# elavoie/non-iid-topology-simulator

Hardware: AMD Instinct MI355X
Metric: param-GB/s mixed (device-resident), 1000-node d-cliques, P=1M fp32 (higher is better)
Workload: dtype f32; 1 GPU; d-cliques N=1000 (10 cliques x 100, fully-connected interclique, MH weights; topology generated by the reference, seed 1337); n_nodes=1000, p=1048576, kernel=clique, mode=fast, parallelism=single GPU, halo_rows_rank0=0, hipgraph=False, slab_memory=VMM 2 MiB chunks (niidmix_hbm_alloc), slab_layout=column-blocked [1024, 1000, 1024], clique-contiguous rows

## Files before the change

include/niidmix.h:

```cpp
#ifndef NIIDMIX_H
#define NIIDMIX_H

#include <stdint.h>
#include <sys/types.h>

#ifdef __cplusplus
extern "C" {
#endif

#define NIIDMIX_ABI_VERSION 6

enum niidmix_status {
    NIIDMIX_OK = 0,
    NIIDMIX_EINVAL = 1,
    NIIDMIX_EALIAS = 2,
    NIIDMIX_EHIP = 3,
    NIIDMIX_EUNSUPPORTED = 4
};

enum niidmix_mode {
    NIIDMIX_MODE_EXACT = 0,
    NIIDMIX_MODE_FAST = 1
};

#define NIIDMIX_FLAG_AVERAGE_ONLY 2

#define NIIDMIX_FLAG_LOW_DEGREE 4

#define NIIDMIX_FLAG_MEAN 8

int niidmix_abi_version(void);

const char *niidmix_last_error(void);

int niidmix_mix_csr_f32(const float *x, int64_t ld_x, float *y, int64_t ld_y, int64_t n_rows,
                        int64_t p, const int64_t *row_ptr, const int32_t *col, const float *val,
                        int mode, void *stream);

int niidmix_mix_ell_f32(const float *x, int64_t ld_x, float *y, int64_t ld_y, int64_t n_rows,
                        int64_t p, int k, const int32_t *ell_col, const float *ell_val,
                        const int32_t *ell_len, int mode, void *stream);

int niidmix_mix_band_f32(const float *x, int64_t ld_x, float *y, int64_t ld_y, int64_t n_rows,
                         int64_t p, int k, int band, const int32_t *ell_col, const float *ell_val,
// ... 174 lines not shown
```

non-iid-topology-simulator_amd/csrc/niidmix.hip:

```cpp
#include <hip/hip_runtime.h>
#include <rccl/rccl.h>

#include <dlfcn.h>
#include <stdarg.h>
#include <stdlib.h>
#include <stdint.h>
#include <stdio.h>
#include <string.h>
#include <sys/types.h>

#include <mutex>
#include <unordered_map>
#include <type_traits>
#include <vector>

#include "../../include/niidmix.h"

typedef float floatx16 __attribute__((ext_vector_type(16)));

namespace {

thread_local char g_last_error[512] = "";

int set_error(int code, const char *fmt, ...) {
// ... 2377 lines not shown
#define NIIDMIX_SEG_REMOTE NIIDMIX_SEG_REMOTE_M("0xfff")
#define NIIDMIX_SEG_REMOTE8 NIIDMIX_SEG_REMOTE_M("7")
#define NIIDMIX_SEG_REMOTE_M(MASK)                                                                   \
    "s_bitcmp1_b32 s41, 29\n\t"                                                                     \
    "s_cbranch_scc0 .Lw_lds_%=\n\t"                                                                 \
    "s_and_b32 s46, s41, " MASK "\n\t"                                                              \
    "s_lshl_b32 s46, s46, 1\n\t"                                                                    \
    "s_set_gpr_idx_on s46, gpr_idx(SRC0)\n\t"                                                       \
    "v_mov_b32 %[q0], v64\n\t"                                                                      \
    "v_mov_b32 %[q1], v65\n\t"                                                                      \
    "s_set_gpr_idx_off\n\t"                                                                         \
    "s_branch .Lw_mskgo_%=\n"                                                                       \
    ".Lw_lds_%=:\n\t"
#define NIIDMIX_REM_IN , [rem] "{v[64:95]}"(rem)
#define NIIDMIX_REM_IN8 , [rem] "{v[64:79]}"(rem)
#define NIIDMIX_SEG_WALK(UPD, MSK) NIIDMIX_SEG_WALK_X(UPD, MSK, "", )
#define NIIDMIX_SEG_LOOP(S, UPD)                                                                     \
    ".Lseg_loop" S "_%=:\n\t"                                                                       \
    NIIDMIX_SEG_POS("%[x0]", "%[x2]", "o2", S "0", UPD)                                              \
    NIIDMIX_SEG_POS("%[x1]", "%[x3]", "o3", S "1", UPD)                                              \
    NIIDMIX_SEG_POS("%[x2]", "%[x0]", "o4", S "2", UPD)                                              \
    NIIDMIX_SEG_POS("%[x3]", "%[x1]", "o5", S "3", UPD)                                              \
    "v_add_u32 %[va], %[o4], %[va]\n\t"                                                             \
    "s_branch .Lseg_loop" S "_%=\n\t"                                                               \
    NIIDMIX_SEG_SKIPBLK("%[x0]", S "0", UPD)                                                         \
    NIIDMIX_SEG_SKIPBLK("%[x1]", S "1", UPD)                                                         \
    NIIDMIX_SEG_SKIPBLK("%[x2]", S "2", UPD)                                                         \
    NIIDMIX_SEG_SKIPBLK("%[x3]", S "3", UPD)
#define NIIDMIX_SEG_WALK_X(UPD, MSK, RMSK, RIN)                                                      \
    asm volatile("s_mov_b32 s36, %[sb0]\n"                                                           \
                 ".Lc_next_%=:\n\t"                                                                  \
                 "s_cmp_ge_u32 s36, %[sb1]\n\t"                                                      \
                 "s_cbranch_scc1 .Lw_end_%=\n\t"                                                     \
                 "s_sub_u32 s37, %[sb1], s36\n\t"                                                    \
                 "s_min_u32 s37, s37, 64\n\t"                                                        \
                 "s_sub_u32 s35, s37, 1\n\t"                                                         \
                 "v_min_u32 %[vo], %[ln], s35\n\t"                                                   \
                 "v_add_u32 %[vo], s36, %[vo]\n\t"                                                   \
                 "v_lshlrev_b32 %[vo], 4, %[vo]\n\t"                                                 \
                 "global_load_dword %[dx], %[vo], %[sp]\n\t"                                         \
                 "global_load_dword %[dy], %[vo], %[sp] offset:4\n\t"                                \
                 "global_load_dword %[dz], %[vo], %[sp] offset:8\n\t"                                \
                 "s_waitcnt vmcnt(0)\n\t"                                                            \
                 "s_mov_b32 s40, 0\n"                                                                \
                 ".Lw_next_%=:\n\t"                                                                  \
                 "s_cmp_ge_u32 s40, s37\n\t"                                                         \
                 "s_cbranch_scc1 .Lc_done_%=\n\t"                                                    \
                 "v_readlane_b32 s41, %[dx], s40\n\t"                                                \
                 "v_readlane_b32 s42, %[dy], s40\n\t"                                                \
                 "v_readlane_b32 s43, %[dz], s40\n\t"                                                \
                 "s_add_u32 s40, s40, 1\n\t"                                                         \
                 "s_and_b32 s39, s41, 0xfff\n\t"                                                     \
                 "s_mul_i32 s39, s39, %[o1]\n\t"                                                     \
                 "s_add_u32 s39, s39, %[base]\n\t"                                                   \
                 "v_add_u32 %[va], s39, %[l8]\n\t"                                                   \
                 "s_bitcmp1_b32 s41, 30\n\t"                                                         \
                 "s_cbranch_scc1 .Lw_masked_%=\n\t"                                                  \
// ... 31 lines not shown
                 NIIDMIX_SEG_LOOP("n14", UPD##14)                                                    \
                 NIIDMIX_SEG_LOOP("n15", UPD##15)                                                    \
                 NIIDMIX_SEG_LOOP("h", UPD##8)                                                       \
                 NIIDMIX_SEG_LOOP("q", UPD##4)                                                       \
                 "\n.Lw_masked_%=:\n\t"                                                              \
                 RMSK                                                                                \
                 "ds_read_b32 %[q0], %[va]\n\t"                                                      \
                 "ds_read_b32 %[q1], %[va] offset:4\n\t"                                             \
                 "s_waitcnt lgkmcnt(0)\n"                                                             \
                 ".Lw_mskgo_%=:\n\t"                                                                 \
                 MSK                                                                                 \
                 "\n.Lc_done_%=:\n\t"                                                                \
                 "s_add_u32 s36, s36, 64\n\t"                                                        \
                 "s_branch .Lc_next_%=\n"                                                            \
                 ".Lw_end_%=:\n\t"                                                                   \
                 "s_waitcnt lgkmcnt(0)"                                                              \
                 : "+{v[32:63]}"(acc), [x0] "=&v"(x0), [x1] "=&v"(x1), [x2] "=&v"(x2),             \
                   [x3] "=&v"(x3), [pr] "=&v"(pr), [sv] "=&v"(sv),                                   \
                   [q0] "=&v"(q0), [q1] "=&v"(q1), [va] "=&v"(va), [dx] "=&v"(dx), [dy] "=&v"(dy),  \
                   [dz] "=&v"(dz), [vo] "=&v"(vo)                                                   \
                 : [sp] "s"(segp), [sb0] "s"(sb0), [sb1] "s"(sb1), [ln] "v"(lane), [base] "s"(base), \
                   [w0] "s"(w0), [w1] "s"(w1), [l8] "v"(lane8), [nr] "s"(nr), [o1] "i"(RB),            \
                   [o2] "i"(2 * RB), [o3] "i"(3 * RB), [o4] "i"(4 * RB), [o5] "i"(5 * RB) RIN         \
                 : "s35", "s36", "s37", "s38", "s39", "s40", "s41", "s42", "s43", "s44", "s45", "s46", \
                   "s47", "m0", "scc", "memory")
template <bool EXACT, int RB>
__device__ __forceinline__ void tlds16_walk(Acc16 &acc, const int32_t *segp, int sb0, int sb1, int base,
                                            int w0, int w1, int lane8, int lane, int nr) {
    static_assert(5 * RB < 65536, "ds_read immediate offset");
    uint64_t x0, x1, x2, x3, pr;
    uint64_t sv;
    uint32_t q0, q1, va, dx, dy, dz, vo;
    if constexpr (EXACT) NIIDMIX_SEG_WALK(NIIDMIX_SEG_UPD_EXACT, NIIDMIX_MSK_EXACT);
    else NIIDMIX_SEG_WALK(NIIDMIX_UPD_FAST, NIIDMIX_MSK_FAST);
    (void)pr;
}
typedef float Rem32 __attribute__((ext_vector_type(32)));
typedef float Rem16 __attribute__((ext_vector_type(16)));
template <int NREM> struct RemRegs { typedef Rem32 V; };
template <> struct RemRegs<8> { typedef Rem16 V; };
template <bool EXACT, int RB, int NREM>
__device__ __forceinline__ void tlds16_walk_rem(Acc16 &acc, const int32_t *segp, int sb0, int sb1,
                                                int base, int w0, int w1, int lane8, int lane,
                                                int nr, const typename RemRegs<NREM>::V &rem) {
    static_assert(5 * RB < 65536, "ds_read immediate offset");
    static_assert(NREM == 8 || NREM == 16, "8 or 16 register rows");
    uint64_t x0, x1, x2, x3, pr;
    uint64_t sv;
    uint32_t q0, q1, va, dx, dy, dz, vo;
    if constexpr (EXACT && NREM == 16)
        NIIDMIX_SEG_WALK_X(NIIDMIX_SEG_UPD_EXACT, NIIDMIX_MSK_EXACT, NIIDMIX_SEG_REMOTE, NIIDMIX_REM_IN);
    else if constexpr (NREM == 16)
        NIIDMIX_SEG_WALK_X(NIIDMIX_UPD_FAST, NIIDMIX_MSK_FAST, NIIDMIX_SEG_REMOTE, NIIDMIX_REM_IN);
    else if constexpr (EXACT)
        NIIDMIX_SEG_WALK_X(NIIDMIX_SEG_UPD_EXACT, NIIDMIX_MSK_EXACT, NIIDMIX_SEG_REMOTE8, NIIDMIX_REM_IN8);
    else
        NIIDMIX_SEG_WALK_X(NIIDMIX_UPD_FAST, NIIDMIX_MSK_FAST, NIIDMIX_SEG_REMOTE8, NIIDMIX_REM_IN8);
    (void)pr;
}

template <bool EXACT>
__device__ __forceinline__ void tlds16_init(Acc16 &acc, int d_slot, int d_ws, int rb, int base, int lane8) {
    uint64_t x0, x1, t, pr;
    uint32_t va;
    if constexpr (EXACT)
        asm volatile("s_mov_b64 s[46:47], 0\n\t"
                 "v_readlane_b32 s40, %[ds], 0\n\t""v_readlane_b32 s42, %[dw], 0\n\t""s_mul_i32 s40, s40, %[rb]\n\t""s_add_u32 s40, s40, %[base]\n\t""v_add_u32 %[va], s40, %[l8]\n\t""ds_read_b64 %[x0], %[va]\n\t"
                 "v_readlane_b32 s40, %[ds], 1\n\t""v_readlane_b32 s44, %[dw], 1\n\t""s_mul_i32 s40, s40, %[rb]\n\t""s_add_u32 s40, s40, %[base]\n\t""v_add_u32 %[va], s40, %[l8]\n\t""ds_read_b64 %[x1], %[va]\n\t"
                 "s_waitcnt lgkmcnt(1)\n\t""v_pk_mul_f32 %[t], %[x0], s[46:47]\n\t""v_pk_mul_f32 %[pr], %[x0], s[42:43] op_sel_hi:[1,0]\n\t""v_pk_add_f32 v[32:33], %[t], %[pr]\n\t"
                 "v_readlane_b32 s40, %[ds], 2\n\t""v_readlane_b32 s42, %[dw], 2\n\t""s_mul_i32 s40, s40, %[rb]\n\t""s_add_u32 s40, s40, %[base]\n\t""v_add_u32 %[va], s40, %[l8]\n\t""ds_read_b64 %[x0], %[va]\n\t"
                 "s_waitcnt lgkmcnt(1)\n\t""v_pk_mul_f32 %[t], %[x1], s[46:47]\n\t""v_pk_mul_f32 %[pr], %[x1], s[44:45] op_sel_hi:[1,0]\n\t""v_pk_add_f32 v[34:35], %[t], %[pr]\n\t"
                 "v_readlane_b32 s40, %[ds], 3\n\t""v_readlane_b32 s44, %[dw], 3\n\t""s_mul_i32 s40, s40, %[rb]\n\t""s_add_u32 s40, s40, %[base]\n\t""v_add_u32 %[va], s40, %[l8]\n\t""ds_read_b64 %[x1], %[va]\n\t"
// ... 101 lines not shown
#endif
#ifndef NIIDMIX_MF_SPLIT
#define NIIDMIX_MF_SPLIT 0
#endif
#ifndef NIIDMIX_TLDS_GLDS
#define NIIDMIX_TLDS_GLDS 1
#endif
inline size_t tlds_slack(bool seg, int cw) {
    const size_t spare = seg ? 2 * (size_t)cw * sizeof(float) : 0;
    return NIIDMIX_TLDS_GLDS && spare < 1024 ? 1024 - spare : 0;
}
constexpr int tile_lds_max_waves(int rt) { return rt == 8 ? 16 : rt == 16 ? 12 : 4; }

template <bool B> struct BoolC { static constexpr bool value = B; };

template <bool EXACT, int RT, int SV, int RS, bool SEG, int NREM = 0, bool MF = false, bool REM2 = false>
__global__ __launch_bounds__(64 * tile_lds_max_waves(RT)) void k_mix_tile_lds(
    const float *__restrict__ x, int64_t ld_x, float *__restrict__ y, int64_t ld_y, int64_t p,
    int64_t n_grp, const int32_t *__restrict__ grp_tile_ptr, const int32_t *__restrict__ grp_src_ptr,
    const int32_t *__restrict__ grp_src_rows, const int64_t *__restrict__ sub_ptr,
    const int32_t *__restrict__ sub_rows, const int32_t *__restrict__ sub_slot,
    const float *__restrict__ sub_wself, const int32_t *__restrict__ pos_slot,
    const uint32_t *__restrict__ pos_mask, const float *__restrict__ pos_w, int tl_flags,
    const int32_t *__restrict__ seg_ptr, const int32_t *__restrict__ seg,
    const float *__restrict__ seg_w, const int32_t *__restrict__ mf_ptr,
    const int32_t *__restrict__ mf, int mf_waves, const int32_t *__restrict__ rem_rows) {
    constexpr int rs = RS;
    const bool avg_only = (tl_flags & 1) != 0;
    const bool small_loops = (tl_flags & 2) == 0;
    constexpr int64_t CW = 2 * RS;
    constexpr uint32_t FULL = (uint32_t)((1ull << RT) - 1ull);
// ... 295 lines not shown
#pragma unroll
            for (int r = 0; r < RT; ++r) {
                const f2 xs = stage[__builtin_amdgcn_readlane(d_slot, r) * rs + sl];
                const float ws = __int_as_float(__builtin_amdgcn_readlane(__float_as_int(d_ws), r));
                acc.set(r, axpy2<EXACT>(ws, xs, xs * 0.f));
            }
        }
        if constexpr (SEG && RT == 16 && NIIDMIX_TLDS_ASM && (NIIDMIX_TLDS_SPLIT == 0 || NIIDMIX_TLDS_SPLIT == 2)) {
            {
                const int sb0 = seg_ptr[sub], sb1 = seg_ptr[sub + 1];
                const int w0 = __float_as_int(seg_w[2 * sub]), w1 = __float_as_int(seg_w[2 * sub + 1]);
                const uint64_t used = __ballot(lane < RT && d_row >= 0);
                const int hi = used ? 64 - __builtin_clzll(used) : 1;
                const int nr = __builtin_amdgcn_readfirstlane(
                    !small_loops ? 16 : hi <= 4 ? 4 : hi <= 8 ? 8 : hi);
                if constexpr (REM && REM2) {
                    int sm = sb1;
                    for (int b = sb0; b < sb1; b += kWave) {
                        const int i = b + lane;
                        const int dx = i < sb1 ? seg[4 * i] : 0;
                        const uint64_t hit = __ballot((dx & (3 << 29)) == (3 << 29) && (dx & 0xfff) >= 8);
                        if (hit) { sm = b + __builtin_ctzll(hit); break; }
                    }
                    tlds16_walk_rem<EXACT, rs * (int)sizeof(f2), 8>(acc.v[0], seg, sb0, sm, (int)lds_base,
                                                                     w0, w1, lane8, lane, nr, rem);
                    if (sm < sb1) {
                        const int sl_ = lane < rs ? lane : rs - 1;
                        const int64_t cr = c0 + 2 * sl_ < p ? c0 + 2 * sl_ : c0;
#pragma unroll
                        for (int r = 0; r < 8; ++r) {
                            const int row = rem_rows[sub * 16 + 8 + r];
// ... 1821 lines not shown
    const int64_t n_chunks = (p + cw - 1) / cw;
    const int64_t n_sub_groups = (plan->n_sub + 3) / 4;
    const int64_t n_items = n_sub_groups * ((n_chunks + 7) / 8) * 8;
    auto kfn = pick<true, false>(mode == NIIDMIX_MODE_EXACT, [&](auto E) { return pick<8, 16, 32>(plan->rt, [&](auto R) {
        return pick<4, 2>(ne, [&](auto N) { return pick<4, 2, 1>(vw, [&](auto V) {
            return k_mix_tile<E(), V(), V() == 4 ? 4 : N(), R()>; }); }); }); });
    hipLaunchKernelGGL(kfn, dim3((unsigned)grid_for(n_items)), dim3(256), 0, s, x, ld_x, y, ld_y, p,
                       plan->n_sub, plan->sub_ptr, plan->sub_rows, plan->sub_wself, plan->pos_src,
                       plan->pos_mask, plan->pos_w, n_sub_groups, n_items, avg_only);
    return check_launch("k_mix_tile");
}

int niidmix_mix_tile_lds_f32(const float *x, int64_t ld_x, float *y, int64_t ld_y, int64_t n_rows,
                             int64_t p, const niidmix_tile_lds_plan *plan, int mode, void *stream) {
    if (!plan) return set_error(NIIDMIX_EINVAL, "null plan");
    int avg_only = strip_flags(&mode, NIIDMIX_FLAG_AVERAGE_ONLY) ? 1 : 0;
    if (int rc = check_mode(mode)) return rc;
    if (env_int("NIIDMIX_TLDS_SMALL", 1) == 0) avg_only |= 2;
    if (p < 0 || plan->n_grp < 0) return set_error(NIIDMIX_EINVAL, "negative size");
    if (plan->rt != 8 && plan->rt != 16 && plan->rt != 32)
        return set_error(NIIDMIX_EUNSUPPORTED, "tile of %d rows (8, 16 or 32 supported)", plan->rt);
    if (plan->n_grp == 0 || p == 0) return NIIDMIX_OK;
    if (!x || !y || !plan->grp_tile_ptr || !plan->grp_src_ptr || !plan->grp_src_rows ||
        !plan->sub_ptr || !plan->sub_rows || !plan->sub_slot || !plan->sub_wself ||
        !plan->pos_slot || !plan->pos_mask || !plan->pos_w)
        return set_error(NIIDMIX_EINVAL, "null pointer");
    if (int rc = check_ld(ld_x, ld_y, p)) return rc;
    if (ld_x >= (1LL << 30)) return set_error(NIIDMIX_EUNSUPPORTED, "ld_x >= 2^30");
    if (n_rows < 1) return set_error(NIIDMIX_EINVAL, "n_rows < 1");
    if (int rc = check_overlap(x, ld_x, y, ld_y, n_rows, p)) return rc;
    if (plan->max_src < 1 || plan->max_src > 256)
        return set_error(NIIDMIX_EUNSUPPORTED, "group with %d source rows (1..256 supported)", plan->max_src);
    const int max_waves = tile_lds_max_waves(plan->rt);
    if (plan->max_tiles < 1 || plan->max_tiles > max_waves)
        return set_error(NIIDMIX_EUNSUPPORTED, "group with %d tiles of %d rows (1..%d supported)",
                         plan->max_tiles, plan->rt, max_waves);
    if (vec_width({p, ld_x, ld_y}, {x, y}) == 1)
        return set_error(NIIDMIX_EUNSUPPORTED, "LDS tile kernel needs even p, ld and 8-B aligned slabs");
    const int sv = vec_width({p, ld_x}, {x}) == 4 ? 4 : 2;
    hipStream_t s = reinterpret_cast<hipStream_t>(stream);
    int cw = 128;
    const size_t lds_cu = 160 * 1024;
    const bool seg = plan->rt == 16 && plan->seg_ptr != nullptr;
    if (seg && (!plan->seg || !plan->seg_w)) return set_error(NIIDMIX_EINVAL, "null segment arrays");
    const bool mf = seg && mode == NIIDMIX_MODE_EXACT && plan->mf_ptr != nullptr;
    const bool rem = plan->rem_rows != nullptr;
    if (rem && (!seg || plan->mf_ptr != nullptr))
        return set_error(NIIDMIX_EINVAL, "rem_rows needs the segment walker (seg_ptr set, mf_ptr NULL)");
    if (rem && plan->rem_regs != 0 && plan->rem_regs != 8 && plan->rem_regs != 16 && plan->rem_regs != -16)
        return set_error(NIIDMIX_EINVAL, "rem_regs %d (0, 8, 16 or -16)", plan->rem_regs);
    if (mf && !plan->mf) return set_error(NIIDMIX_EINVAL, "null MFMA position list");
    const int variant = !seg ? 0 : !rem ? (mf ? 2 : 1) : plan->rem_regs == 8 ? 4 : plan->rem_regs == -16 ? 5 : 3;
    const int mf_waves = env_int("NIIDMIX_TLDS_MF_WAVES", plan->max_tiles);
    const int stage_rows = plan->max_src + (seg ? 2 : 0);
    if (plan->rt == 16) {
        auto blocks = [&](int c) {
            const size_t per = (size_t)stage_rows * c * sizeof(float) + tlds_slack(seg, c);
            const size_t b = per ? lds_cu / per : 3;
            return (int)(b < 3 ? b : 3);
        };
        const int target = blocks(96);
        for (int c : {128, 120, 96})
            if (blocks(c) >= target) { cw = c; break; }
    }
    cw = env_int("NIIDMIX_TLDS_COLS", cw, {128, 120, 96});
    const int64_t n_chunks = (p + cw - 1) / cw;
    const int64_t n_items = (int64_t)plan->n_grp * ((n_chunks + 7) / 8) * 8;
    if (n_items > 0x7fffffffLL) return set_error(NIIDMIX_EUNSUPPORTED, "too many (group, chunk) items");
    const size_t lds = (size_t)stage_rows * cw * sizeof(float) + tlds_slack(seg, cw);
    auto kfn = pick<true, false>(mode == NIIDMIX_MODE_EXACT, [&](auto E) { return pick<8, 16, 32>(plan->rt, [&](auto R) {
        return pick<4, 2>(sv, [&](auto V) { return pick<64, 60, 48>(cw / 2, [&](auto RS) {
            return pick<0, 1, 2, 3, 4, 5>(variant, [&](auto T) {
                constexpr int t = R() == 16 ? T() : 0;
                return k_mix_tile_lds<E(), R(), V(), RS(), (t > 0), (t == 3 ? 16 : t >= 4 ? 8 : 0), (E() && t == 2), (t == 5)>;
            }); }); }); }); });
    if (lds > 65536) if (int rc = lds_opt_in(kfn, lds, "k_mix_tile_lds")) return rc;
    hipLaunchKernelGGL(kfn, dim3((unsigned)n_items), dim3((unsigned)(64 * plan->max_tiles)), lds, s, x, ld_x,
                       y, ld_y, p, (int64_t)plan->n_grp, plan->grp_tile_ptr, plan->grp_src_ptr,
                       plan->grp_src_rows, plan->sub_ptr, plan->sub_rows, plan->sub_slot, plan->sub_wself,
                       plan->pos_slot, plan->pos_mask, plan->pos_w, avg_only, seg ? plan->seg_ptr : nullptr,
                       plan->seg, plan->seg_w, mf ? plan->mf_ptr : nullptr, plan->mf, mf_waves,
                       plan->rem_rows);
    return check_launch("k_mix_tile_lds");
}

int niidmix_mix_dense_f32(const float *x, int64_t ld_x, float *y, int64_t ld_y, int64_t n,
                          int64_t p, const float *w, const int64_t *row_ptr, const int32_t *col,
                          const float *val, void *stream) {
    if (n < 0 || p < 0) return set_error(NIIDMIX_EINVAL, "negative size");
// ... 646 lines not shown
```

non-iid-topology-simulator_amd/niidmix/ops.py:

```python
import ctypes
import os
from typing import Optional

import numpy as np
import torch

from . import _lib
from .factor import build_clique_plan
from .tile import (LDS_MAX_WAVES, balanced_tile_rows, build_tile_lds_plan, build_tile_mfma_positions,
                   build_tile_plan, build_tile_segments, rem_two_phase)
from .topology import MixCSR, to_csr

EXACT, FAST = _lib.MODE_EXACT, _lib.MODE_FAST
AVERAGE_ONLY = 2
LOW_DEGREE = 4
MEAN = 8
MEMBER_GATEWAY = 256


def _stream(t):
    return ctypes.c_void_p(torch.cuda.current_stream(t.device).cuda_stream)


def _req(cond, msg):
    if not cond:
        raise RuntimeError(msg)


def _slab(name, t, rows=None, cols=None):
# ... 257 lines not shown
                          sub_wself.data_ptr(), pos_src.data_ptr() or some,
                          pos_mask.data_ptr() or some, pos_w.data_ptr() or some)
    rc = _lib.lib.niidmix_mix_tile_f32(x.data_ptr(), _ld(x), out.data_ptr(), _ld(out), out.shape[0],
                                       x.shape[1], ctypes.byref(plan), int(mode), _stream(x))
    _lib.check(rc, "niidmix::mix_tile")


@torch.library.custom_op("niidmix::mix_tile_lds", mutates_args=("out",))
def mix_tile_lds(x: torch.Tensor, sub_ptr: torch.Tensor, sub_rows: torch.Tensor,
                 sub_slot: torch.Tensor, sub_wself: torch.Tensor, pos_slot: torch.Tensor,
                 pos_mask: torch.Tensor, pos_w: torch.Tensor, grp_tile_ptr: torch.Tensor,
                 grp_src_ptr: torch.Tensor, grp_src_rows: torch.Tensor, out: torch.Tensor, rt: int,
                 max_src: int, max_tiles: int, mode: int, seg_ptr: Optional[torch.Tensor] = None,
                 seg: Optional[torch.Tensor] = None, seg_w: Optional[torch.Tensor] = None,
                 mf_ptr: Optional[torch.Tensor] = None, mf: Optional[torch.Tensor] = None,
                 rem_rows: Optional[torch.Tensor] = None, rem_regs: int = 16) -> None:
    _slab("x", x)
    _slab("out", out, cols=x.shape[1])
    dev = x.device
    t = sub_ptr.numel() - 1
    g = grp_tile_ptr.numel() - 1
    _vec("sub_ptr", sub_ptr, torch.int64, dev)
    _vec("sub_rows", sub_rows, torch.int32, dev, t * rt)
    _vec("sub_slot", sub_slot, torch.int32, dev, t * rt)
    _vec("sub_wself", sub_wself, torch.float32, dev, t * rt)
    _vec("pos_slot", pos_slot, torch.int32, dev)
    _vec("pos_mask", pos_mask, torch.int32, dev, pos_slot.numel())
    _vec("pos_w", pos_w, torch.float32, dev, pos_slot.numel() * rt)
    _vec("grp_tile_ptr", grp_tile_ptr, torch.int32, dev)
    _vec("grp_src_ptr", grp_src_ptr, torch.int32, dev, g + 1)
    _vec("grp_src_rows", grp_src_rows, torch.int32, dev)
# ... 6 lines not shown
        _req(seg.numel() % 4 == 0 and seg.data_ptr() % 16 == 0, "seg: [S, 4] int32, 16-B aligned")
        _vec("seg_w", seg_w, torch.float32, dev, 2 * t)
        segs = (seg_ptr.data_ptr(), seg.data_ptr(), seg_w.data_ptr())
    mfs = (None, None)
    if mf_ptr is not None:
        _req(seg_ptr is not None and mf is not None, "MFMA position lists: with the segments, mf_ptr and mf")
        _vec("mf_ptr", mf_ptr, torch.int32, dev, t + 1)
        _vec("mf", mf, torch.int32, dev)
        _req(mf.numel() % 4 == 0 and mf.data_ptr() % 16 == 0, "mf: [E, 4] int32, 16-B aligned")
        mfs = (mf_ptr.data_ptr(), mf.data_ptr() if mf.numel() else mf_ptr.data_ptr())
    rem = None
    if rem_rows is not None:
        _req(seg_ptr is not None and mf_ptr is None,
             "register rows: with the segments and without the MFMA position lists")
        _vec("rem_rows", rem_rows, torch.int32, dev, t * 16)
        _req(rem_regs in (8, 16, -16), f"rem_regs {rem_regs} (8, 16 or -16)")
        rem = rem_rows.data_ptr()
    _no_overlap(x, out)
    some = sub_ptr.data_ptr()
    plan = _lib.TileLdsPlanC(t, int(rt), g, int(max_src), int(max_tiles), sub_ptr.data_ptr(),
                             sub_rows.data_ptr(), sub_slot.data_ptr(), sub_wself.data_ptr(),
                             pos_slot.data_ptr() or some, pos_mask.data_ptr() or some,
                             pos_w.data_ptr() or some, grp_tile_ptr.data_ptr(),
                             grp_src_ptr.data_ptr(), grp_src_rows.data_ptr(), *segs, *mfs, rem,
                             int(rem_regs) if rem is not None else 0)
    rc = _lib.lib.niidmix_mix_tile_lds_f32(x.data_ptr(), _ld(x), out.data_ptr(), _ld(out),
                                           out.shape[0], x.shape[1], ctypes.byref(plan), int(mode),
                                           _stream(x))
    _lib.check(rc, "niidmix::mix_tile_lds")


@torch.library.custom_op("niidmix::mix_dense", mutates_args=("out",))
def mix_dense(x: torch.Tensor, w: torch.Tensor, row_ptr: torch.Tensor, col: torch.Tensor,
              val: torch.Tensor, out: torch.Tensor) -> None:
    _slab("x", x)
    n = x.shape[0]
    _slab("out", out, rows=n, cols=x.shape[1])
    _req(w.device == x.device and w.dtype == torch.float32 and w.shape == (n, n) and
         w.is_contiguous(), "w: expected contiguous fp32 [N, N] (W[src, dst])")
    _vec("row_ptr", row_ptr, torch.int64, x.device, n + 1)
    _vec("col", col, torch.int32, x.device)
    _vec("val", val, torch.float32, x.device, col.numel())
# ... 274 lines not shown
        Cin, H, W, C, scratch.data_ptr(), nbytes, _stream(theta))
    _lib.check(rc, "niidmix::gnlenet_eval_rows")


_LAZY = {
    "plan": "clique", "plan_reason": "clique", "p_clique_ptr": "clique", "p_member_row": "clique",
    "p_member_group": "clique", "p_coef": "clique", "p_res_ptr": "clique", "p_res_col": "clique",
    "p_res_val": "clique", "p_res_member": "clique",
    "tile": "tile", "tile_reason": "tile", "t_sub_ptr": "tile", "t_sub_rows": "tile",
    "t_sub_wself": "tile", "t_pos_src": "tile", "t_pos_mask": "tile", "t_pos_w": "tile",
    "tlds": "tlds", "tlds_reason": "tlds", "l_sub_ptr": "tlds", "l_sub_rows": "tlds",
    "l_sub_slot": "tlds", "l_sub_wself": "tlds", "l_pos_slot": "tlds", "l_pos_mask": "tlds",
    "l_pos_w": "tlds", "l_grp_tile_ptr": "tlds", "l_grp_src_ptr": "tlds", "l_grp_src_rows": "tlds",
    "tseg": "tlds", "s_seg_ptr": "tlds", "s_seg": "tlds", "s_seg_w": "tlds",
    "tmf": "tlds", "m_mf_ptr": "tlds", "m_mf": "tlds", "l_rem_rows": "tlds", "tlds_rem2": "tlds",
    "w_dense": "dense", "w_split": "dense",
    "ell": "ell", "e_col": "ell", "e_val": "ell", "e_len": "ell", "band": "ell",
}


class _Scratch:

    def __init__(self, owner):
        self._owner = owner

    def __getattr__(self, name):
        return getattr(self._owner, name)


class Mixer:
# ... 139 lines not shown
        self.l_sub_wself = torch.from_numpy(tp.sub_wself).to(dev)
        self.l_pos_slot = torch.from_numpy(lp.pos_slot).to(dev)
        self.l_pos_mask = torch.from_numpy(tp.pos_mask.view(np.int32)).to(dev)
        self.l_pos_w = torch.from_numpy(tp.pos_w).to(dev)
        self.l_grp_tile_ptr = torch.from_numpy(lp.grp_tile_ptr).to(dev)
        self.l_grp_src_ptr = torch.from_numpy(lp.grp_src_ptr).to(dev)
        self.l_grp_src_rows = torch.from_numpy(lp.grp_src_rows).to(dev)
        self.tseg = ts
        if ts is not None:
            self.s_seg_ptr = torch.from_numpy(ts.seg_ptr).to(dev)
            self.s_seg = torch.from_numpy(np.ascontiguousarray(ts.seg).reshape(-1)).to(dev)
            self.s_seg_w = torch.from_numpy(np.ascontiguousarray(ts.seg_w).reshape(-1)).to(dev)
        self.l_rem_rows = (torch.from_numpy(lp.rem_rows).to(dev) if lp.rem_rows is not None
                           else None)
        self.tlds_rem2 = lp.rem_regs == 16 and ts is not None and rem_two_phase(lp, ts)
        self.tmf = tm if ts is not None else None
        if self.tmf is not None:
            self.m_mf_ptr = torch.from_numpy(tm.mf_ptr).to(dev)
            self.m_mf = torch.from_numpy(np.ascontiguousarray(tm.mf).reshape(-1)).to(dev)

    def _build_ell(self):
        lay = self._hosted("ell", lambda: ell_layout(self.csr))
        self.ell = None if lay is None else lay[0]
        self.band = None if lay is None else self._hosted("band", lambda: band_of(self.csr, lay[0]))
        if lay is not None:
            k, col, val, ln = lay
            self.e_col = torch.from_numpy(col).to(self.device)
            self.e_val = torch.from_numpy(val).to(self.device)
            self.e_len = torch.from_numpy(ln).to(self.device)

# ... 113 lines not shown
            _req(self.tlds is not None, f"no LDS tile plan: {self.tlds_reason}")
            lp = self.tlds
            ts = self.tseg
            segs = (self.s_seg_ptr, self.s_seg, self.s_seg_w) if \
                self.use_segments and ts is not None and ts.lp is lp else ()
            rem = None
            if lp.rem_rows is not None:
                _req(bool(segs), "a plan with register rows needs the segment walker "
                     "(use_segments; NIIDMIX_TLDS_REMOTE=0 builds a plan without them)")
                rem = self.l_rem_rows
            if segs and rem is None and k == "tile-lds-exact" and self.use_mfma and \
                    self.tmf is not None and self.tmf.lp is lp:
                segs = segs + (self.m_mf_ptr, self.m_mf)
            if rem is not None:
                two = self.tlds_rem2 and os.environ.get("NIIDMIX_TLDS_REM2", "1") == "1"
                segs = segs + (None, None, rem, -16 if two else lp.rem_regs)
            mix_tile_lds(x, self.l_sub_ptr, self.l_sub_rows, self.l_sub_slot, self.l_sub_wself,
                         self.l_pos_slot, self.l_pos_mask, self.l_pos_w, self.l_grp_tile_ptr,
                         self.l_grp_src_ptr, self.l_grp_src_rows, out, lp.tile.rt, lp.max_src,
                         lp.max_tiles, EXACT if k == "tile-lds-exact" else FAST, *segs)
        elif k == "clique":
            _req(self.plan is not None, f"no clique plan: {self.plan_reason}")
            mix_clique(x, *self._clique_args(), out, self.plan.max_clique,
                       self.plan.max_clique_res)
        elif k == "dense":
            _req(b6_fits(self.n, x), "kernel 'dense' (bf16x6): 16 rows of the slab or the "
                 "split W exceed 2^31 B; use 'dense-f32'")
            mix_dense_b6(x, self.w_split, self.row_ptr, self.col, self.val, out)
        elif k == "dense-f32":
            mix_dense(x, self.w_dense, self.row_ptr, self.col, self.val, out)
        else:
# ... 31 lines not shown
```

non-iid-topology-simulator_amd/niidmix/tile.py:

```python
import bisect
import os
from dataclasses import dataclass

import numpy as np

TILE_ROWS = (8, 16, 32)
POS_UNIFORM = 1 << 30


@dataclass
class TilePlan:
    rt: int
    sub_ptr: np.ndarray
    sub_rows: np.ndarray
    sub_wself: np.ndarray
    pos_src: np.ndarray
    pos_mask: np.ndarray
    pos_w: np.ndarray
    nnz: int
    grp_tile_ptr: np.ndarray = None

    @property
    def n_sub(self):
        return len(self.sub_ptr) - 1
# ... 423 lines not shown
                    cur[3] |= 1 << (i - 32)
            if skip >= 0:
                if cur[8] is None:
                    cur[6] = skip
                if i < 32:
                    cur[4] |= 1 << i
                else:
                    cur[5] |= 1 << (i - 32)
                cur[8] = skip + 1
            cur[1] += 1
        if cur is not None:
            segs.append(cur)
        seg_ptr.append(len(segs))
        seg_w.append(ws)
    arr = np.zeros((len(segs), SEG_WORDS), np.int64)
    for i, sg in enumerate(segs):
        if sg[0] == "M":
            _, slot, cm, wb = sg
            arr[i] = [slot | SEG_HARD, cm, wb, 0]
        else:
            s0, ln, wlo, _, klo, _, r0 = sg[:7]
            arr[i] = [s0 | (ln << 12) | (r0 << 20), wlo, klo, 0]
    arr = (arr & 0xFFFFFFFF).astype(np.uint32).view(np.int32)
    return TileSegments(seg_ptr=np.asarray(seg_ptr, np.int32), seg=arr.reshape(-1, SEG_WORDS),
                        seg_w=np.asarray(seg_w, np.float32).reshape(-1, 2), lp=lp)


def rem_two_phase(lp, ts):
    if lp.rem_rows is None or ts is None or ts.lp is not lp:
        return False
    w0 = np.asarray(ts.seg)[:, 0].astype(np.int64)
    rem = ((w0 & SEG_HARD) != 0) & ((w0 & SEG_REMOTE) != 0)
    high = rem & ((w0 & SEG_SLOT) >= 8)
    low = rem & ((w0 & SEG_SLOT) < 8)
    for t in range(lp.tile.n_sub):
        b, e = int(ts.seg_ptr[t]), int(ts.seg_ptr[t + 1])
        h = np.flatnonzero(high[b:e])
        if len(h) and np.any(low[b + h[0]:e]):
            return False
    return True


def segments_row_lists(lp, ts):
    tp = lp.tile
    rt = tp.rt
    src_rows = lp.grp_src_rows
    gtp = lp.grp_tile_ptr
    grp_of = np.zeros(tp.n_sub, np.int64)
    for gi in range(len(gtp) - 1):
        grp_of[gtp[gi]:gtp[gi + 1]] = gi
    out = {}
    seg = ts.seg.view(np.uint32).astype(np.int64)
    for t in range(tp.n_sub):
        base = int(lp.grp_src_ptr[grp_of[t]])
        rows = tp.sub_rows[t * rt:(t + 1) * rt]
        lists = {r: [(int(rows[r]), np.float32(tp.sub_wself[t * rt + r]))]
                 for r in range(rt) if rows[r] >= 0}
        w0, w1 = ts.seg_w[t]
        for s in seg[ts.seg_ptr[t]:ts.seg_ptr[t + 1]]:
            hd = int(s[0])
            if hd & SEG_HARD:
                if hd & SEG_REMOTE:
                    src = int(lp.rem_rows[t * REM_MAX + (hd & SEG_SLOT)])
                else:
                    src = int(src_rows[base + (hd & SEG_SLOT)])
                m, w = int(s[1]), np.uint32(s[2]).view(np.float32)
                for r in lists:
                    if (m >> r) & 1:
                        lists[r].append((src, np.float32(w)))
                continue
            s0, ln, r_skip = hd & SEG_SLOT, (hd >> 12) & 0xff, (hd >> 20) & 0xff
            wsel, skip = int(s[1]), int(s[2])
            for i in range(ln):
                src = int(src_rows[base + s0 + i])
                w = w1 if (wsel >> i) & 1 else w0
                skipped = -1
                if (skip >> i) & 1:
# ... 83 lines not shown
```

Baseline: 2989 GB/s.

## Stream remote register rows through an 8-slot ring with prefetched next rows

```diff
diff --git a/include/niidmix.h b/include/niidmix.h
--- a/include/niidmix.h
+++ b/include/niidmix.h
@@ -28,6 +28,8 @@
 #define NIIDMIX_FLAG_LOW_DEGREE 4
 
 #define NIIDMIX_FLAG_MEAN 8
+
+#define NIIDMIX_FLAG_REM_ORDERED 16
 
 int niidmix_abi_version(void);
 
diff --git a/non-iid-topology-simulator_amd/csrc/niidmix.hip b/non-iid-topology-simulator_amd/csrc/niidmix.hip
--- a/non-iid-topology-simulator_amd/csrc/niidmix.hip
+++ b/non-iid-topology-simulator_amd/csrc/niidmix.hip
@@ -2415,7 +2415,57 @@
     ".Lw_lds_%=:\n\t"
 #define NIIDMIX_REM_IN , [rem] "{v[64:95]}"(rem)
 #define NIIDMIX_REM_IN8 , [rem] "{v[64:79]}"(rem)
-#define NIIDMIX_SEG_WALK(UPD, MSK) NIIDMIX_SEG_WALK_X(UPD, MSK, "", )
+#define NIIDMIX_REMS_LD(D, K)                                                                        \
+    "\n.Lrs_ld" K "_%=:\n\t"                                                                        \
+    "global_load_dwordx2 " D ", %[vf], s[38:39]\n\t"                                               \
+    "s_branch .Lw_mskgo_%=\n"
+#define NIIDMIX_SEG_REMOTE_S                                                                         \
+    "s_bitcmp1_b32 s41, 29\n\t"                                                                     \
+    "s_cbranch_scc0 .Lw_lds_%=\n\t"                                                                 \
+    "s_and_b32 s46, s41, 7\n\t"                                                                     \
+    "s_lshl_b32 s46, s46, 1\n\t"                                                                    \
+    "s_waitcnt vmcnt(7)\n\t"                                                                        \
+    "s_set_gpr_idx_on s46, gpr_idx(SRC0)\n\t"                                                       \
+    "v_mov_b32 %[q0], v64\n\t"                                                                      \
+    "v_mov_b32 %[q1], v65\n\t"                                                                      \
+    "s_set_gpr_idx_off\n\t"                                                                         \
+    "s_sub_u32 s47, s40, 1\n\t"                                                                     \
+    "v_readlane_b32 s47, %[dw], s47\n\t"                                                            \
+    "s_max_i32 s47, s47, 0\n\t"                                                                     \
+    "s_mul_hi_u32 s39, s47, %[ldx]\n\t"                                                             \
+    "s_mul_i32 s38, s47, %[ldx]\n\t"                                                                \
+    "s_add_u32 s38, s38, %[xlo]\n\t"                                                                \
+    "s_addc_u32 s39, s39, %[xhi]\n\t"                                                               \
+    "s_bitcmp1_b32 s46, 3\n\t"                                                                      \
+    "s_cbranch_scc1 .Lrs_hi_%=\n\t"                                                                 \
+    "s_bitcmp1_b32 s46, 2\n\t"                                                                      \
+    "s_cbranch_scc1 .Lrs_23_%=\n\t"                                                                 \
+    "s_bitcmp1_b32 s46, 1\n\t"                                                                      \
+    "s_cbranch_scc1 .Lrs_ld1_%=\n\t"                                                                \
+    "s_branch .Lrs_ld0_%=\n"                                                                        \
+    ".Lrs_23_%=:\n\t"                                                                               \
+    "s_bitcmp1_b32 s46, 1\n\t"                                                                      \
+    "s_cbranch_scc1 .Lrs_ld3_%=\n\t"                                                                \
+    "s_branch .Lrs_ld2_%=\n"                                                                        \
+    ".Lrs_hi_%=:\n\t"                                                                               \
+    "s_bitcmp1_b32 s46, 2\n\t"                                                                      \
+    "s_cbranch_scc1 .Lrs_67_%=\n\t"                                                                 \
+    "s_bitcmp1_b32 s46, 1\n\t"                                                                      \
+    "s_cbranch_scc1 .Lrs_ld5_%=\n\t"                                                                \
+    "s_branch .Lrs_ld4_%=\n"                                                                        \
+    ".Lrs_67_%=:\n\t"                                                                               \
+    "s_bitcmp1_b32 s46, 1\n\t"                                                                      \
+    "s_cbranch_scc1 .Lrs_ld7_%=\n\t"                                                                \
+    "s_branch .Lrs_ld6_%=\n"                                                                        \
+    NIIDMIX_REMS_LD("v[64:65]", "0") NIIDMIX_REMS_LD("v[66:67]", "1")                              \
+    NIIDMIX_REMS_LD("v[68:69]", "2") NIIDMIX_REMS_LD("v[70:71]", "3")                              \
+    NIIDMIX_REMS_LD("v[72:73]", "4") NIIDMIX_REMS_LD("v[74:75]", "5")                              \
+    NIIDMIX_REMS_LD("v[76:77]", "6") NIIDMIX_REMS_LD("v[78:79]", "7")                              \
+    ".Lw_lds_%=:\n\t"
+#define NIIDMIX_REMS_DW "global_load_dword %[dw], %[vo], %[sp] offset:12\n\t"
+#define NIIDMIX_REMS_OUT , [rem] "+{v[64:79]}"(rem), [dw] "=&v"(dw)
+#define NIIDMIX_REMS_IN , [xlo] "s"(xlo), [xhi] "s"(xhi), [ldx] "s"(ldx4), [vf] "v"(voff)
+#define NIIDMIX_SEG_WALK(UPD, MSK) NIIDMIX_SEG_WALK_Y(UPD, MSK, "", , "", , "")
 #define NIIDMIX_SEG_LOOP(S, UPD)                                                                     \
     ".Lseg_loop" S "_%=:\n\t"                                                                       \
     NIIDMIX_SEG_POS("%[x0]", "%[x2]", "o2", S "0", UPD)                                              \
@@ -2428,7 +2478,7 @@
     NIIDMIX_SEG_SKIPBLK("%[x1]", S "1", UPD)                                                         \
     NIIDMIX_SEG_SKIPBLK("%[x2]", S "2", UPD)                                                         \
     NIIDMIX_SEG_SKIPBLK("%[x3]", S "3", UPD)
-#define NIIDMIX_SEG_WALK_X(UPD, MSK, RMSK, RIN)                                                      \
+#define NIIDMIX_SEG_WALK_Y(UPD, MSK, RMSK, RIN, XLD, ROUT, XEND)                                     \
     asm volatile("s_mov_b32 s36, %[sb0]\n"                                                           \
                  ".Lc_next_%=:\n\t"                                                                  \
                  "s_cmp_ge_u32 s36, %[sb1]\n\t"                                                      \
@@ -2442,6 +2492,7 @@
                  "global_load_dword %[dx], %[vo], %[sp]\n\t"                                         \
                  "global_load_dword %[dy], %[vo], %[sp] offset:4\n\t"                                \
                  "global_load_dword %[dz], %[vo], %[sp] offset:8\n\t"                                \
+                 XLD                                                                                 \
                  "s_waitcnt vmcnt(0)\n\t"                                                            \
                  "s_mov_b32 s40, 0\n"                                                                \
                  ".Lw_next_%=:\n\t"                                                                  \
@@ -2503,11 +2554,12 @@
                  "s_add_u32 s36, s36, 64\n\t"                                                        \
                  "s_branch .Lc_next_%=\n"                                                            \
                  ".Lw_end_%=:\n\t"                                                                   \
+                 XEND                                                                                \
                  "s_waitcnt lgkmcnt(0)"                                                              \
                  : "+{v[32:63]}"(acc), [x0] "=&v"(x0), [x1] "=&v"(x1), [x2] "=&v"(x2),             \
                    [x3] "=&v"(x3), [pr] "=&v"(pr), [sv] "=&v"(sv),                                   \
                    [q0] "=&v"(q0), [q1] "=&v"(q1), [va] "=&v"(va), [dx] "=&v"(dx), [dy] "=&v"(dy),  \
-                   [dz] "=&v"(dz), [vo] "=&v"(vo)                                                   \
+                   [dz] "=&v"(dz), [vo] "=&v"(vo) ROUT                                              \
                  : [sp] "s"(segp), [sb0] "s"(sb0), [sb1] "s"(sb1), [ln] "v"(lane), [base] "s"(base), \
                    [w0] "s"(w0), [w1] "s"(w1), [l8] "v"(lane8), [nr] "s"(nr), [o1] "i"(RB),            \
                    [o2] "i"(2 * RB), [o3] "i"(3 * RB), [o4] "i"(4 * RB), [o5] "i"(5 * RB) RIN         \
@@ -2538,13 +2590,30 @@
     uint64_t sv;
     uint32_t q0, q1, va, dx, dy, dz, vo;
     if constexpr (EXACT && NREM == 16)
-        NIIDMIX_SEG_WALK_X(NIIDMIX_SEG_UPD_EXACT, NIIDMIX_MSK_EXACT, NIIDMIX_SEG_REMOTE, NIIDMIX_REM_IN);
+        NIIDMIX_SEG_WALK_Y(NIIDMIX_SEG_UPD_EXACT, NIIDMIX_MSK_EXACT, NIIDMIX_SEG_REMOTE, NIIDMIX_REM_IN, "", , "");
     else if constexpr (NREM == 16)
-        NIIDMIX_SEG_WALK_X(NIIDMIX_UPD_FAST, NIIDMIX_MSK_FAST, NIIDMIX_SEG_REMOTE, NIIDMIX_REM_IN);
+        NIIDMIX_SEG_WALK_Y(NIIDMIX_UPD_FAST, NIIDMIX_MSK_FAST, NIIDMIX_SEG_REMOTE, NIIDMIX_REM_IN, "", , "");
     else if constexpr (EXACT)
-        NIIDMIX_SEG_WALK_X(NIIDMIX_SEG_UPD_EXACT, NIIDMIX_MSK_EXACT, NIIDMIX_SEG_REMOTE8, NIIDMIX_REM_IN8);
+        NIIDMIX_SEG_WALK_Y(NIIDMIX_SEG_UPD_EXACT, NIIDMIX_MSK_EXACT, NIIDMIX_SEG_REMOTE8, NIIDMIX_REM_IN8, "", , "");
     else
-        NIIDMIX_SEG_WALK_X(NIIDMIX_UPD_FAST, NIIDMIX_MSK_FAST, NIIDMIX_SEG_REMOTE8, NIIDMIX_REM_IN8);
+        NIIDMIX_SEG_WALK_Y(NIIDMIX_UPD_FAST, NIIDMIX_MSK_FAST, NIIDMIX_SEG_REMOTE8, NIIDMIX_REM_IN8, "", , "");
+    (void)pr;
+}
+template <bool EXACT, int RB>
+__device__ __forceinline__ void tlds16_walk_rems(Acc16 &acc, const int32_t *segp, int sb0, int sb1,
+                                                 int base, int w0, int w1, int lane8, int lane, int nr,
+                                                 Rem16 &rem, uint32_t xlo, uint32_t xhi, uint32_t ldx4,
+                                                 uint32_t voff) {
+    static_assert(5 * RB < 65536, "ds_read immediate offset");
+    uint64_t x0, x1, x2, x3, pr;
+    uint64_t sv;
+    uint32_t q0, q1, va, dx, dy, dz, vo, dw;
+    if constexpr (EXACT)
+        NIIDMIX_SEG_WALK_Y(NIIDMIX_SEG_UPD_EXACT, NIIDMIX_MSK_EXACT, NIIDMIX_SEG_REMOTE_S, NIIDMIX_REMS_IN,
+                           NIIDMIX_REMS_DW, NIIDMIX_REMS_OUT, "s_waitcnt vmcnt(0)\n\t");
+    else
+        NIIDMIX_SEG_WALK_Y(NIIDMIX_UPD_FAST, NIIDMIX_MSK_FAST, NIIDMIX_SEG_REMOTE_S, NIIDMIX_REMS_IN,
+                           NIIDMIX_REMS_DW, NIIDMIX_REMS_OUT, "s_waitcnt vmcnt(0)\n\t");
     (void)pr;
 }
 
@@ -2676,7 +2745,8 @@
 
 template <bool B> struct BoolC { static constexpr bool value = B; };
 
-template <bool EXACT, int RT, int SV, int RS, bool SEG, int NREM = 0, bool MF = false, bool REM2 = false>
+template <bool EXACT, int RT, int SV, int RS, bool SEG, int NREM = 0, bool MF = false, bool REM2 = false,
+          bool REMS = false>
 __global__ __launch_bounds__(64 * tile_lds_max_waves(RT)) void k_mix_tile_lds(
     const float *__restrict__ x, int64_t ld_x, float *__restrict__ y, int64_t ld_y, int64_t p,
     int64_t n_grp, const int32_t *__restrict__ grp_tile_ptr, const int32_t *__restrict__ grp_src_ptr,
@@ -3002,7 +3072,16 @@
                 const int hi = used ? 64 - __builtin_clzll(used) : 1;
                 const int nr = __builtin_amdgcn_readfirstlane(
                     !small_loops ? 16 : hi <= 4 ? 4 : hi <= 8 ? 8 : hi);
-                if constexpr (REM && REM2) {
+                if constexpr (REM && REMS) {
+                    const int sl_ = lane < rs ? lane : rs - 1;
+                    const uint32_t voff = c0 + 2 * sl_ < p ? (uint32_t)(2 * sl_) * 4u : 0u;
+                    const uint64_t xb = reinterpret_cast<uint64_t>(x + c0);
+                    tlds16_walk_rems<EXACT, rs * (int)sizeof(f2)>(
+                        acc.v[0], seg, sb0, sb1, (int)lds_base, w0, w1, lane8, lane, nr, rem,
+                        __builtin_amdgcn_readfirstlane((uint32_t)xb),
+                        __builtin_amdgcn_readfirstlane((uint32_t)(xb >> 32)),
+                        __builtin_amdgcn_readfirstlane((uint32_t)ld_x * 4u), voff);
+                } else if constexpr (REM && REM2) {
                     int sm = sb1;
                     for (int b = sb0; b < sb1; b += kWave) {
                         const int i = b + lane;
@@ -4854,9 +4933,11 @@
 int niidmix_mix_tile_lds_f32(const float *x, int64_t ld_x, float *y, int64_t ld_y, int64_t n_rows,
                              int64_t p, const niidmix_tile_lds_plan *plan, int mode, void *stream) {
     if (!plan) return set_error(NIIDMIX_EINVAL, "null plan");
-    int avg_only = strip_flags(&mode, NIIDMIX_FLAG_AVERAGE_ONLY) ? 1 : 0;
+    const int flags = strip_flags(&mode, NIIDMIX_FLAG_AVERAGE_ONLY | NIIDMIX_FLAG_REM_ORDERED);
+    int avg_only = (flags & NIIDMIX_FLAG_AVERAGE_ONLY) ? 1 : 0;
     if (int rc = check_mode(mode)) return rc;
     if (env_int("NIIDMIX_TLDS_SMALL", 1) == 0) avg_only |= 2;
+    if (flags & NIIDMIX_FLAG_REM_ORDERED) avg_only |= 4;
     if (p < 0 || plan->n_grp < 0) return set_error(NIIDMIX_EINVAL, "negative size");
     if (plan->rt != 8 && plan->rt != 16 && plan->rt != 32)
         return set_error(NIIDMIX_EUNSUPPORTED, "tile of %d rows (8, 16 or 32 supported)", plan->rt);
@@ -4887,10 +4968,16 @@
     const bool rem = plan->rem_rows != nullptr;
     if (rem && (!seg || plan->mf_ptr != nullptr))
         return set_error(NIIDMIX_EINVAL, "rem_rows needs the segment walker (seg_ptr set, mf_ptr NULL)");
-    if (rem && plan->rem_regs != 0 && plan->rem_regs != 8 && plan->rem_regs != 16 && plan->rem_regs != -16)
-        return set_error(NIIDMIX_EINVAL, "rem_regs %d (0, 8, 16 or -16)", plan->rem_regs);
+    if (rem && plan->rem_regs != 0 && plan->rem_regs != 8 && plan->rem_regs != 16 && plan->rem_regs != -16 &&
+        plan->rem_regs != -8)
+        return set_error(NIIDMIX_EINVAL, "rem_regs %d (0, 8, 16, -16 or -8)", plan->rem_regs);
+    if (rem && plan->rem_regs < 0 && !(avg_only & 4))
+        return set_error(NIIDMIX_EINVAL, "rem_regs %d needs NIIDMIX_FLAG_REM_ORDERED in mode: the plan's "
+                         "register-row order validated (niidmix.tile.rem_two_phase / rem_streamed)",
+                         plan->rem_regs);
     if (mf && !plan->mf) return set_error(NIIDMIX_EINVAL, "null MFMA position list");
-    const int variant = !seg ? 0 : !rem ? (mf ? 2 : 1) : plan->rem_regs == 8 ? 4 : plan->rem_regs == -16 ? 5 : 3;
+    const int variant = !seg ? 0 : !rem ? (mf ? 2 : 1) : plan->rem_regs == 8 ? 4 : plan->rem_regs == -16 ? 5
+                        : plan->rem_regs == -8 ? 6 : 3;
     const int mf_waves = env_int("NIIDMIX_TLDS_MF_WAVES", plan->max_tiles);
     const int stage_rows = plan->max_src + (seg ? 2 : 0);
     if (plan->rt == 16) {
@@ -4910,9 +4997,10 @@
     const size_t lds = (size_t)stage_rows * cw * sizeof(float) + tlds_slack(seg, cw);
     auto kfn = pick<true, false>(mode == NIIDMIX_MODE_EXACT, [&](auto E) { return pick<8, 16, 32>(plan->rt, [&](auto R) {
         return pick<4, 2>(sv, [&](auto V) { return pick<64, 60, 48>(cw / 2, [&](auto RS) {
-            return pick<0, 1, 2, 3, 4, 5>(variant, [&](auto T) {
+            return pick<0, 1, 2, 3, 4, 5, 6>(variant, [&](auto T) {
                 constexpr int t = R() == 16 ? T() : 0;
-                return k_mix_tile_lds<E(), R(), V(), RS(), (t > 0), (t == 3 ? 16 : t >= 4 ? 8 : 0), (E() && t == 2), (t == 5)>;
+                return k_mix_tile_lds<E(), R(), V(), RS(), (t > 0), (t == 3 ? 16 : t >= 4 ? 8 : 0), (E() && t == 2), (t == 5),
+                                      (t == 6)>;
             }); }); }); }); });
     if (lds > 65536) if (int rc = lds_opt_in(kfn, lds, "k_mix_tile_lds")) return rc;
     hipLaunchKernelGGL(kfn, dim3((unsigned)n_items), dim3((unsigned)(64 * plan->max_tiles)), lds, s, x, ld_x,
diff --git a/non-iid-topology-simulator_amd/niidmix/ops.py b/non-iid-topology-simulator_amd/niidmix/ops.py
--- a/non-iid-topology-simulator_amd/niidmix/ops.py
+++ b/non-iid-topology-simulator_amd/niidmix/ops.py
@@ -8,11 +8,12 @@
 from . import _lib
 from .factor import build_clique_plan
 from .tile import (LDS_MAX_WAVES, balanced_tile_rows, build_tile_lds_plan, build_tile_mfma_positions,
-                   build_tile_plan, build_tile_segments, rem_two_phase)
+                   build_tile_plan, build_tile_segments, rem_streamed, rem_two_phase)
 from .topology import MixCSR, to_csr
 
 EXACT, FAST = _lib.MODE_EXACT, _lib.MODE_FAST
 AVERAGE_ONLY = 2
+FLAG_REM_ORDERED = 16
 LOW_DEGREE = 4
 MEAN = 8
 MEMBER_GATEWAY = 256
@@ -300,7 +301,8 @@
                  max_src: int, max_tiles: int, mode: int, seg_ptr: Optional[torch.Tensor] = None,
                  seg: Optional[torch.Tensor] = None, seg_w: Optional[torch.Tensor] = None,
                  mf_ptr: Optional[torch.Tensor] = None, mf: Optional[torch.Tensor] = None,
-                 rem_rows: Optional[torch.Tensor] = None, rem_regs: int = 16) -> None:
+                 rem_rows: Optional[torch.Tensor] = None, rem_regs: int = 16,
+                 rem_ordered: bool = False) -> None:
     _slab("x", x)
     _slab("out", out, cols=x.shape[1])
     dev = x.device
@@ -337,7 +339,7 @@
         _req(seg_ptr is not None and mf_ptr is None,
              "register rows: with the segments and without the MFMA position lists")
         _vec("rem_rows", rem_rows, torch.int32, dev, t * 16)
-        _req(rem_regs in (8, 16, -16), f"rem_regs {rem_regs} (8, 16 or -16)")
+        _req(rem_regs in (8, 16, -16, -8), f"rem_regs {rem_regs} (8, 16, -16 or -8)")
         rem = rem_rows.data_ptr()
     _no_overlap(x, out)
     some = sub_ptr.data_ptr()
@@ -348,7 +350,8 @@
                              grp_src_ptr.data_ptr(), grp_src_rows.data_ptr(), *segs, *mfs, rem,
                              int(rem_regs) if rem is not None else 0)
     rc = _lib.lib.niidmix_mix_tile_lds_f32(x.data_ptr(), _ld(x), out.data_ptr(), _ld(out),
-                                           out.shape[0], x.shape[1], ctypes.byref(plan), int(mode),
+                                           out.shape[0], x.shape[1], ctypes.byref(plan),
+                                           int(mode) | (FLAG_REM_ORDERED if rem_ordered else 0),
                                            _stream(x))
     _lib.check(rc, "niidmix::mix_tile_lds")
 
@@ -653,6 +656,7 @@
     "l_pos_w": "tlds", "l_grp_tile_ptr": "tlds", "l_grp_src_ptr": "tlds", "l_grp_src_rows": "tlds",
     "tseg": "tlds", "s_seg_ptr": "tlds", "s_seg": "tlds", "s_seg_w": "tlds",
     "tmf": "tlds", "m_mf_ptr": "tlds", "m_mf": "tlds", "l_rem_rows": "tlds", "tlds_rem2": "tlds",
+    "tlds_rems": "tlds",
     "w_dense": "dense", "w_split": "dense",
     "ell": "ell", "e_col": "ell", "e_val": "ell", "e_len": "ell", "band": "ell",
 }
@@ -822,6 +826,8 @@
         self.l_rem_rows = (torch.from_numpy(lp.rem_rows).to(dev) if lp.rem_rows is not None
                            else None)
         self.tlds_rem2 = lp.rem_regs == 16 and ts is not None and rem_two_phase(lp, ts)
+        self.tlds_rems = self.tlds_rem2 and rem_streamed(lp, ts) and \
+            os.environ.get("NIIDMIX_TLDS_REMS", "1") != "0"
         self.tmf = tm if ts is not None else None
         if self.tmf is not None:
             self.m_mf_ptr = torch.from_numpy(tm.mf_ptr).to(dev)
@@ -965,7 +971,8 @@
                 segs = segs + (self.m_mf_ptr, self.m_mf)
             if rem is not None:
                 two = self.tlds_rem2 and os.environ.get("NIIDMIX_TLDS_REM2", "1") == "1"
-                segs = segs + (None, None, rem, -16 if two else lp.rem_regs)
+                segs = segs + (None, None, rem,
+                               (-8 if self.tlds_rems else -16) if two else lp.rem_regs, two)
             mix_tile_lds(x, self.l_sub_ptr, self.l_sub_rows, self.l_sub_slot, self.l_sub_wself,
                          self.l_pos_slot, self.l_pos_mask, self.l_pos_w, self.l_grp_tile_ptr,
                          self.l_grp_src_ptr, self.l_grp_src_rows, out, lp.tile.rt, lp.max_src,
diff --git a/non-iid-topology-simulator_amd/niidmix/tile.py b/non-iid-topology-simulator_amd/niidmix/tile.py
--- a/non-iid-topology-simulator_amd/niidmix/tile.py
+++ b/non-iid-topology-simulator_amd/niidmix/tile.py
@@ -461,10 +461,15 @@
         seg_ptr.append(len(segs))
         seg_w.append(ws)
     arr = np.zeros((len(segs), SEG_WORDS), np.int64)
+    tile_of = np.repeat(np.arange(tp.n_sub), np.diff(seg_ptr))
     for i, sg in enumerate(segs):
         if sg[0] == "M":
             _, slot, cm, wb = sg
-            arr[i] = [slot | SEG_HARD, cm, wb, 0]
+            nxt = 0
+            if slot & SEG_REMOTE:
+                ri = (slot & SEG_SLOT) + 8
+                nxt = int(lp.rem_rows[tile_of[i] * REM_MAX + ri]) if ri < REM_MAX else -1
+            arr[i] = [slot | SEG_HARD, cm, wb, nxt]
         else:
             s0, ln, wlo, _, klo, _, r0 = sg[:7]
             arr[i] = [s0 | (ln << 12) | (r0 << 20), wlo, klo, 0]
@@ -488,7 +493,28 @@
     return True
 
 
-def segments_row_lists(lp, ts):
+def rem_streamed(lp, ts):
+    if lp.rem_rows is None or ts is None or ts.lp is not lp:
+        return False
+    seg = np.asarray(ts.seg)
+    w0 = seg[:, 0].astype(np.int64)
+    rem = ((w0 & SEG_HARD) != 0) & ((w0 & SEG_REMOTE) != 0)
+    rows = np.asarray(lp.rem_rows).reshape(-1, REM_MAX)
+    for t in range(lp.tile.n_sub):
+        b, e = int(ts.seg_ptr[t]), int(ts.seg_ptr[t + 1])
+        at = b + np.flatnonzero(rem[b:e])
+        k = int((rows[t] >= 0).sum())
+        if len(at) != k or np.any(rows[t, :k] < 0) or \
+                not np.array_equal(w0[at] & SEG_SLOT, np.arange(k)):
+            return False
+        want = np.full(k, -1, np.int64)
+        want[:max(k - 8, 0)] = rows[t, 8:k]
+        if not np.array_equal(seg[at, 3], want):
+            return False
+    return True
+
+
+def segments_row_lists(lp, ts, streamed=False):
     tp = lp.tile
     rt = tp.rt
     src_rows = lp.grp_src_rows
@@ -504,10 +530,15 @@
         lists = {r: [(int(rows[r]), np.float32(tp.sub_wself[t * rt + r]))]
                  for r in range(rt) if rows[r] >= 0}
         w0, w1 = ts.seg_w[t]
+        slots = ([max(int(v), 0) for v in lp.rem_rows[t * REM_MAX:t * REM_MAX + 8]]
+                 if streamed and lp.rem_rows is not None else None)
         for s in seg[ts.seg_ptr[t]:ts.seg_ptr[t + 1]]:
             hd = int(s[0])
             if hd & SEG_HARD:
-                if hd & SEG_REMOTE:
+                if hd & SEG_REMOTE and slots is not None:
+                    src = slots[hd & 7]
+                    slots[hd & 7] = max(int(np.int64(s[3]).astype(np.int32)), 0)
+                elif hd & SEG_REMOTE:
                     src = int(lp.rem_rows[t * REM_MAX + (hd & SEG_SLOT)])
                 else:
                     src = int(src_rows[base + (hd & SEG_SLOT)])
```

Measured after the change: 2987 GB/s. About the same (-0.0%).
